# senweaver/senweaver-ide

Measured on AMD Instinct MI355X. Metric: APO iterations/sec (beam=4, llama-3-8b scorer, bf16), higher is better.
Workload: dtype bf16; 1 GPU; model=llama-3-8b, global_batch=64, seq_len=2048, parallelism=dp1, beam_width=4, branch_factor=4, gradient_batch_size=4

## Files before the change

### senweaver_amd/models/llama.py

```python

from __future__ import annotations

import math
import os
from typing import TYPE_CHECKING, Callable, List, Optional

import torch

from .. import ops
from .config import ModelConfig

if TYPE_CHECKING:
    from ..engine.kvcache import PagedKVCache


class LlamaModel:
    def __init__(self, config: ModelConfig, device="cpu", dtype=torch.bfloat16, seed: int = 0,
                 tp=None, quant: str = "bf16", ep=None):
        from ..parallel.tp import TPContext, shard_gateup, shard_qkv, shard_rows
        from ..parallel.ep import EPContext
        self.config = config
        self.device = torch.device(device)
        self.dtype = dtype
        self.tp = tp if tp is not None else TPContext()
# ... 168 lines not shown
    def plan_tensors(self, plan):
        cache = self._plan_cache
        key = (plan.S, plan.owner, plan.skip)
        hit = cache.get(key)
        if hit is None:
            if len(cache) >= 64:
                cache.clear()
            pos = torch.cat([torch.arange(plan.skip[b], plan.S)
                             for b in range(plan.B)])
            row = torch.repeat_interleave(
                torch.arange(plan.B),
                torch.tensor([plan.S - s for s in plan.skip]))
            hit = tuple(t.to(self.device) for t in (
                torch.tensor(plan.skip, dtype=torch.int32),
                torch.tensor(plan.base, dtype=torch.int32),
                torch.tensor(plan.owner, dtype=torch.int32),
                pos.to(torch.int32), row * plan.S + pos))
            cache[key] = hit
        return hit

    def prefill_packed(self, tokens: torch.Tensor, plan) -> torch.Tensor:
        c = self.config
        B, S = tokens.shape
        skip, base, owner, positions, flat_idx = self.plan_tensors(plan)
        Tp = plan.Tp
        if plan.is_identity or (self.device.type == "cuda"
                                and (S % 128 != 0 or S < 256)):
            return self.prefill(tokens).reshape(B * S, -1)[flat_idx]

        def attend(li, L, qkv):
            qb, kb = ops.rope_scatter_qkv_packed(
                qkv, self.cos_sin, positions, self.local_heads,
                self.local_kv_heads, c.head_dim, B, S, skip, base, owner)
            vt = ops.vt_from_qkv_packed(qkv, self.local_heads,
                                        self.local_kv_heads, c.head_dim, B, S,
                                        skip, base, owner)
            attn = ops.attn_fwd_packed(qb, kb, vt, self.scale, skip, base, Tp,
                                       flat_idx)
            if self.quant == "bf16" and not attn.is_cuda:
                return torch.matmul(attn, L["o"].t())
            return self._linear(attn, L, "o")

        hidden = self.embed[tokens.reshape(B * S)[flat_idx]]
        return self._layers(hidden, attend, full_rows=B * S)

    def _down_rows(self, h: torch.Tensor, L: dict, full_rows: int) -> Optional[int]:
        Tp = h.shape[0]
        if self.quant != "bf16" or "down" not in L or full_rows <= Tp:
            return None
        cache = self._down_rows_cache
        hit = cache.get((Tp, full_rows), 0)
        if hit == 0:
            hit = full_rows
            if h.is_cuda:
                w = L["down"]
                act = torch.empty(full_rows, w.shape[1], dtype=h.dtype,
                                  device=h.device).normal_()
                act[Tp:].zero_()
                t_packed = ops.gemm_lt_best_us(act[:Tp], w)
                t_full = ops.gemm_lt_best_us(act, w)
                if t_packed is not None and t_full is not None:
                    fill = ops.hip_ext().gemm_lt_fill_us(
                        act, (full_rows - Tp) * w.shape[1] * act.element_size())
                    if t_packed <= 1.05 * (t_full + fill):
                        hit = None
                elif torch.cuda.is_current_stream_capturing():
                    return full_rows
            if len(cache) >= 64:
                cache.clear()
            cache[(Tp, full_rows)] = hit
        return hit
# ... 251 lines not shown
```

### senweaver_amd/ops/__init__.py

```python

from __future__ import annotations

import math
import os
import weakref
from typing import Optional

import torch

from . import reference as ref

_ext = None
_ext_err: Optional[str] = None


def _load_ext():
    global _ext, _ext_err
    if _ext is not None or _ext_err is not None:
        return _ext
    from . import build as _build

    try:
        _ext = _build.load_prebuilt()
        if _ext is None:
# ... 112 lines not shown
    src = ref.packed_src_rows_ref(B, S, skip, base, owner).reshape(-1)
    return rope_scatter_qkv(qkv[src], cos_sin, positions[src], Hq, Hk, D, B, S)


def vt_from_qkv_packed(qkv: torch.Tensor, Hq: int, Hk: int, D: int, B: int,
                       S: int, skip, base, owner) -> torch.Tensor:
    if _on_gpu(qkv):
        return hip_ext().vt_from_qkv_packed(qkv.contiguous(), Hq, Hk, D, B, S,
                                            skip, base, owner)
    src = ref.packed_src_rows_ref(B, S, skip, base, owner).reshape(-1)
    return vt_from_qkv(qkv[src], Hq, Hk, D, B, S)


def attn_fwd_t_packed(q: torch.Tensor, k: torch.Tensor, vt: torch.Tensor,
                      scale: float, skip, base, Tp: int, flat_idx) -> torch.Tensor:
    B, H, S, D = q.shape
    if _on_gpu(q) and _ATTN_IMPL != "v2" and ((S + 255) // 256) * B * H >= 512:
        return hip_ext().attn_fwd_v5_packed(q.contiguous(), k.contiguous(),
                                            vt.contiguous(), scale, skip, base,
                                            Tp)
    ot = attn_fwd_t(q, k, vt, scale)
    return ot.permute(1, 2, 0, 3).reshape(H * D, B * S).index_select(1, flat_idx)


def attn_fwd_packed(q: torch.Tensor, k: torch.Tensor, vt: torch.Tensor,
                    scale: float, skip, base, Tp: int, flat_idx) -> torch.Tensor:
    B, H, S, D = q.shape
    if _on_gpu(q) and _ATTN_IMPL != "v2" and ((S + 255) // 256) * B * H >= 512:
        return hip_ext().attn_fwd_v5_packed_rm(q.contiguous(), k.contiguous(),
                                               vt.contiguous(), scale, skip,
                                               base, Tp)
    ot = attn_fwd_t(q, k, vt, scale)
    return ot.permute(0, 3, 1, 2).reshape(B * S, H * D).index_select(0, flat_idx)


def swiglu(gateup: torch.Tensor, out_rows: Optional[int] = None) -> torch.Tensor:
    if out_rows is not None and out_rows > gateup.shape[0]:
        if _on_gpu(gateup):
            return hip_ext().swiglu_padded(gateup.contiguous(), out_rows)
        act = ref.swiglu_ref(gateup)
        return torch.nn.functional.pad(act, (0, 0, 0, out_rows - act.shape[0]))
    if _on_gpu(gateup):
        return hip_ext().swiglu(gateup.contiguous())
    return ref.swiglu_ref(gateup)


_GEMM_IMPL = os.environ.get("SENWEAVER_GEMM", "auto")
_GEMM_TUNE = os.environ.get("SENWEAVER_GEMM_TUNE", "1") != "0"
_ATTN_IMPL = os.environ.get("SENWEAVER_ATTN", "auto")


def swiglu_gemv(gateup: torch.Tensor, w_down: torch.Tensor) -> torch.Tensor:
    K = gateup.shape[-1] // 2
    if (_on_gpu(gateup) and gateup.shape[0] == 1 and K % 1024 == 0
            and 4096 < K <= 14336 and w_down.shape[0] % 8 == 0):
        return hip_ext().swiglu_gemv_bt(gateup.contiguous(), w_down.contiguous())
    act = swiglu(gateup)
    return gemm_bt(act, w_down)


def gemv_fp8w(x: torch.Tensor, w_q: torch.Tensor, w_s: torch.Tensor) -> torch.Tensor:
    K = x.shape[-1]
    if _on_gpu(x) and x.shape[0] <= 8 and K % 1024 == 0 and w_q.shape[0] % 4 == 0:
        return hip_ext().gemv_bt_fp8w(x.contiguous(), w_q.contiguous(),
                                      w_s.contiguous())
    wf = w_q.view(torch.float8_e4m3fn).float() * w_s.unsqueeze(1)
# ... 325 lines not shown
```

### senweaver_amd/ops/csrc/attention_v5.hip

```cpp

#include "common.h"
#include "kernels.h"

typedef __attribute__((ext_vector_type(8))) short short8;
typedef __attribute__((ext_vector_type(16))) float f32x16;

#define V5_KVBLK 64
#define V5_QBLK 256
#define V5_NT 512
#define V5_CHUNKS (V5_KVBLK * 16)
#define V5_KC (V5_CHUNKS / V5_NT)

static __device__ __forceinline__ const ushort* v5_src(
    const ushort* __restrict__ src, long long ld, int chunks_per_row, int row,
    int cl) {
  const int c = (cl ^ row) & (chunks_per_row - 1);
  return src + (long long)row * ld + c * 8;
}

static __device__ __forceinline__ void v5_glds(const ushort* g,
                                               ushort* lds_wave) {
  __builtin_amdgcn_global_load_lds(
      (const __attribute__((address_space(1))) unsigned int*)g,
      (__attribute__((address_space(3))) unsigned int*)lds_wave, 16, 0, 0);
}

static __device__ __forceinline__ short8 v5_read(const ushort* lds_tile,
                                                 int row, int c,
                                                 int chunks_per_row) {
  const int phys = (c ^ row) & (chunks_per_row - 1);
  return *reinterpret_cast<const short8*>(lds_tile + (row * chunks_per_row + phys) * 8);
}

static __device__ __forceinline__ unsigned v5_cvt_pk_bf16(float lo, float hi) {
  unsigned r;
  asm("v_cvt_pk_bf16_f32 %0, %1, %2" : "=v"(r) : "v"(lo), "v"(hi));
  return r;
}

static __device__ __forceinline__ float v5_max(float a, float b) {
  float r;
  asm("v_max_f32 %0, %1, %2" : "=v"(r) : "v"(a), "v"(b));
  return r;
}

static __device__ __forceinline__ float v5_exp2(float x) {
  float r;
  asm("v_exp_f32 %0, %1" : "=v"(r) : "v"(x));
  return r;
}

template <int PACK>
static __device__ __forceinline__ void attn5_body(
    const ushort* __restrict__ Q, const ushort* __restrict__ K,
    const ushort* __restrict__ VT, ushort* __restrict__ OT, int B, int H,
    int Hk, int S, float scale, const int* __restrict__ pk_skip = nullptr,
    const int* __restrict__ pk_base = nullptr, int Tp = 0) {
  const int qb = gridDim.x - 1 - blockIdx.x;
  const int h = blockIdx.y;
  const int b = blockIdx.z;
  int skip = 0;
  if (PACK) {
    skip = pk_skip[b];
    if (qb * V5_QBLK + V5_QBLK <= skip) return;
  }
  const int kvh = h / (H / Hk);
  const int D = 128;

  const ushort* Qh = Q + (((long long)b * H + h) * S) * D;
  const ushort* Kh = K + (((long long)b * Hk + kvh) * S) * D;
  const ushort* VTh = VT + (((long long)b * Hk + kvh) * D) * S;
  ushort* OTh = OT + (((long long)b * H + h) * D) * S;

  const int tid = threadIdx.x;
  const int wid = tid >> 6;
  const int lane = tid & 63;
  const int l31 = lane & 31;
  const int lhi = lane >> 5;
  const int q0 = qb * V5_QBLK + wid * 32;
  const int q_lane = q0 + l31;
  const bool live = q_lane < S;

  __shared__ __attribute__((aligned(16))) ushort smem[2][V5_KVBLK * 128 + 128 * V5_KVBLK];

  short8 qf[8];
  {
    const long long qrow = (long long)(live ? q_lane : 0) * D;
#pragma unroll
    for (int st = 0; st < 8; ++st)
      qf[st] = *reinterpret_cast<const short8*>(Qh + qrow + st * 16 + lhi * 8);
  }

  float m_run = -INFINITY, l_run = 0.f;
  f32x16 o_acc[4];
#pragma unroll
  for (int db = 0; db < 4; ++db)
#pragma unroll
    for (int r = 0; r < 16; ++r) o_acc[db][r] = 0.f;

  const int kv_end = min(S, qb * V5_QBLK + V5_QBLK);
  for (int s0 = 0; s0 < V5_CHUNKS; s0 += V5_NT) {
    const int s = s0 + tid;
    if (s >= V5_CHUNKS) break;
    v5_glds(v5_src(Kh, D, 16, s / 16, s % 16),
            smem[0] + (long long)(s0 + (tid & ~63)) * 8);
  }
  for (int s0 = 0; s0 < V5_CHUNKS; s0 += V5_NT) {
    const int s = s0 + tid;
    if (s >= V5_CHUNKS) break;
    v5_glds(v5_src(VTh, S, 8, s / 8, s % 8),
            smem[0] + V5_KVBLK * 128 + (long long)(s0 + (tid & ~63)) * 8);
  }
  __syncthreads();
  int buf = 0;
  for (int kv0 = 0; kv0 < kv_end; kv0 += V5_KVBLK) {
    const bool more = kv0 + V5_KVBLK < kv_end;
    const ushort* k_lds = smem[buf];
    const ushort* vt_lds = smem[buf] + V5_KVBLK * 128;

    __builtin_amdgcn_s_setprio(1);
    f32x16 st[2];
#pragma unroll
    for (int sub = 0; sub < 2; ++sub) {
      f32x16 acc;
#pragma unroll
      for (int r = 0; r < 16; ++r) acc[r] = 0.f;
#pragma unroll
      for (int stp = 0; stp < 8; ++stp) {
        short8 kf = v5_read(k_lds, sub * 32 + l31, stp * 2 + lhi, 16);
        acc = __builtin_amdgcn_mfma_f32_32x32x16_bf16(kf, qf[stp], acc, 0, 0, 0);
      }
      st[sub] = acc;
    }
    __builtin_amdgcn_s_setprio(0);

    short8 stg[2 * V5_KC];
    if (more) {
      const ushort* Kn = Kh + (long long)(kv0 + V5_KVBLK) * D;
      const ushort* VTn = VTh + kv0 + V5_KVBLK;
#pragma unroll
      for (int c = 0; c < V5_KC; ++c) {
        const int s = tid + c * V5_NT;
        stg[c] = *reinterpret_cast<const short8*>(v5_src(Kn, D, 16, s / 16, s % 16));
        stg[V5_KC + c] = *reinterpret_cast<const short8*>(v5_src(VTn, S, 8, s / 8, s % 8));
      }
    }

    float vals[32];
    float tile_max = -INFINITY;
    const float scl = scale * 1.44269504f;
    const bool interior = kv0 + V5_KVBLK - 1 <= q0;
    if (interior) {
#pragma unroll
      for (int sub = 0; sub < 2; ++sub)
#pragma unroll
        for (int r = 0; r < 16; ++r) {
          const float v = st[sub][r] * scl;
          vals[sub * 16 + r] = v;
          tile_max = v5_max(tile_max, v);
        }
    } else {
#pragma unroll
      for (int sub = 0; sub < 2; ++sub)
#pragma unroll
        for (int r = 0; r < 16; ++r) {
          const int kv = kv0 + sub * 32 + (r & 3) + 8 * (r >> 2) + 4 * lhi;
          float v = st[sub][r] * scl;
          if (kv > q_lane) v = -INFINITY;
          vals[sub * 16 + r] = v;
          tile_max = v5_max(tile_max, v);
        }
    }
    tile_max = v5_max(tile_max, __shfl_xor(tile_max, 32, 64));
    const bool defer = __all((int)(tile_max - m_run <= 11.54f));
    float m_new, alpha;
    if (defer) {
      m_new = m_run;
      alpha = 1.f;
    } else {
      m_new = fmaxf(m_run, tile_max);
      alpha = (m_run == -INFINITY) ? 0.f : v5_exp2(m_run - m_new);
    }
    float rsum = 0.f;
    m_run = m_new;
    if (!defer) {
#pragma unroll
      for (int db = 0; db < 4; ++db)
#pragma unroll
        for (int r = 0; r < 16; ++r) o_acc[db][r] *= alpha;
    }

    if (more) {
      ushort* kd = smem[buf ^ 1];
      ushort* vd = smem[buf ^ 1] + V5_KVBLK * 128;
#pragma unroll
      for (int c = 0; c < V5_KC; ++c) {
        *reinterpret_cast<short8*>(kd + (long long)(tid + c * V5_NT) * 8) = stg[c];
        *reinterpret_cast<short8*>(vd + (long long)(tid + c * V5_NT) * 8) = stg[V5_KC + c];
      }
    }

#pragma unroll
    for (int sub = 0; sub < 2; ++sub) {
#pragma unroll
      for (int g = 0; g < 2; ++g) {
        const int base = sub * 16 + g * 8;
        float p[8];
#pragma unroll
        for (int i = 0; i < 8; ++i) {
          p[i] = v5_exp2(vals[base + i] - m_new);
          rsum += p[i];
        }
        unsigned x0 = v5_cvt_pk_bf16(p[0], p[1]);
        unsigned y0 = v5_cvt_pk_bf16(p[4], p[5]);
        unsigned x1 = v5_cvt_pk_bf16(p[2], p[3]);
        unsigned y1 = v5_cvt_pk_bf16(p[6], p[7]);
        auto r0 = __builtin_amdgcn_permlane32_swap(x0, y0, false, false);
        auto r1 = __builtin_amdgcn_permlane32_swap(x1, y1, false, false);
        short8 pfrag;
        unsigned* pw = reinterpret_cast<unsigned*>(&pfrag);
        pw[0] = (unsigned)r0[0];
        pw[1] = (unsigned)r1[0];
        pw[2] = (unsigned)r0[1];
        pw[3] = (unsigned)r1[1];
        const int kvg = sub * 32 + g * 16;
        __builtin_amdgcn_s_setprio(1);
#pragma unroll
        for (int db = 0; db < 4; ++db) {
          short8 vf = v5_read(vt_lds, db * 32 + l31, (kvg >> 3) + lhi, 8);
          o_acc[db] = __builtin_amdgcn_mfma_f32_32x32x16_bf16(vf, pfrag, o_acc[db], 0, 0, 0);
        }
        __builtin_amdgcn_s_setprio(0);
      }
    }
    rsum += __shfl_xor(rsum, 32, 64);
    l_run = l_run * alpha + rsum;

    __syncthreads();
    buf ^= 1;
  }

  const float inv_l = (l_run > 0.f) ? 1.f / l_run : 0.f;
  if (!live) return;
  if (PACK) {
    const long long col = (long long)pk_base[b] + q_lane;
    if (q_lane < skip || col < 0 || col >= Tp) return;
    if (PACK == 2) {
      ushort* Op = OT + col * ((long long)H * D) + h * D + 4 * lhi;
#pragma unroll
      for (int db = 0; db < 4; ++db)
#pragma unroll
        for (int g = 0; g < 4; ++g) {
          ushort4 v;
          v.x = f2bf(o_acc[db][g * 4 + 0] * inv_l);
          v.y = f2bf(o_acc[db][g * 4 + 1] * inv_l);
          v.z = f2bf(o_acc[db][g * 4 + 2] * inv_l);
          v.w = f2bf(o_acc[db][g * 4 + 3] * inv_l);
          *reinterpret_cast<ushort4*>(Op + db * 32 + 8 * g) = v;
        }
      return;
    }
    ushort* OTp = OT + (long long)h * D * Tp + col;
#pragma unroll
    for (int db = 0; db < 4; ++db)
#pragma unroll
      for (int r = 0; r < 16; ++r) {
        const int d = db * 32 + (r & 3) + 8 * (r >> 2) + 4 * lhi;
        OTp[(long long)d * Tp] = f2bf(o_acc[db][r] * inv_l);
      }
// ... 4 lines not shown
#pragma unroll
    for (int r = 0; r < 16; ++r) {
      const int d = db * 32 + (r & 3) + 8 * (r >> 2) + 4 * lhi;
      OTh[(long long)d * S + q_lane] = f2bf(o_acc[db][r] * inv_l);
    }
}

extern "C" __global__ void __launch_bounds__(512)
attn_fwd_v5_kernel(const ushort* __restrict__ Q, const ushort* __restrict__ K,
                   const ushort* __restrict__ VT, ushort* __restrict__ OT,
                   int B, int H, int Hk, int S, float scale) {
  attn5_body<0>(Q, K, VT, OT, B, H, Hk, S, scale);
}

extern "C" __global__ void __launch_bounds__(512)
attn_fwd_v5_packed_kernel(const ushort* __restrict__ Q,
                          const ushort* __restrict__ K,
                          const ushort* __restrict__ VT,
                          ushort* __restrict__ OT, int B, int H, int Hk,
                          int S, float scale, const int* __restrict__ skip,
                          const int* __restrict__ base, int Tp) {
  attn5_body<1>(Q, K, VT, OT, B, H, Hk, S, scale, skip, base, Tp);
}

extern "C" __global__ void __launch_bounds__(512)
attn_fwd_v5_packed_rm_kernel(const ushort* __restrict__ Q,
                             const ushort* __restrict__ K,
                             const ushort* __restrict__ VT,
                             ushort* __restrict__ O, int B, int H, int Hk,
                             int S, float scale, const int* __restrict__ skip,
                             const int* __restrict__ base, int Tp) {
  attn5_body<2>(Q, K, VT, O, B, H, Hk, S, scale, skip, base, Tp);
}
```

### senweaver_amd/ops/csrc/bindings.hip

```cpp

#include <torch/extension.h>
#include <c10/hip/HIPStream.h>
#include <hip/hip_runtime.h>

#include "common.h"
#include "kernels.h"

namespace {

inline hipStream_t cur_stream() {
  return c10::hip::getCurrentHIPStream().stream();
}

inline const ushort* bf16_ptr(const torch::Tensor& t) {
  return reinterpret_cast<const ushort*>(t.data_ptr());
}
inline ushort* bf16_mut(torch::Tensor& t) {
  return reinterpret_cast<ushort*>(t.data_ptr());
}

void check_bf16(const torch::Tensor& t, const char* name) {
  TORCH_CHECK(t.is_cuda(), name, " must be on GPU");
  TORCH_CHECK(t.scalar_type() == torch::kBFloat16, name, " must be bf16");
  TORCH_CHECK(t.is_contiguous(), name, " must be contiguous");
// ... 587 lines not shown
    ot = *out;
    check_bf16(ot, "out");
    TORCH_CHECK(ot.sizes().vec() == shape, "attn_fwd_v5_packed: out has the wrong shape");
    TORCH_CHECK((uintptr_t)ot.data_ptr() % 16 == 0, "attn_fwd_v5_packed: out must be 16-byte aligned");
  } else {
    ot = torch::empty(shape, q.options());
  }
  const dim3 grid((S + 255) / 256, H, B);
  if (row_major) {
    attn_fwd_v5_packed_rm_kernel<<<grid, dim3(512), 0, cur_stream()>>>(
        bf16_ptr(q), bf16_ptr(k), bf16_ptr(vt), bf16_mut(ot), B, H, Hk, S,
        (float)scale, skip.data_ptr<int>(), base.data_ptr<int>(), (int)Tp);
  } else {
    attn_fwd_v5_packed_kernel<<<grid, dim3(512), 0, cur_stream()>>>(
        bf16_ptr(q), bf16_ptr(k), bf16_ptr(vt), bf16_mut(ot), B, H, Hk, S,
        (float)scale, skip.data_ptr<int>(), base.data_ptr<int>(), (int)Tp);
  }
  HIP_CHECK_KERNEL();
  return ot;
}

torch::Tensor attn_fwd_v5_packed(torch::Tensor q, torch::Tensor k,
                                 torch::Tensor vt, double scale,
                                 torch::Tensor skip, torch::Tensor base,
                                 int64_t Tp) {
  return attn_packed_launch(q, k, vt, scale, skip, base, Tp, false, c10::nullopt);
}

torch::Tensor attn_fwd_v5_packed_rm(torch::Tensor q, torch::Tensor k,
                                    torch::Tensor vt, double scale,
                                    torch::Tensor skip, torch::Tensor base,
                                    int64_t Tp, c10::optional<torch::Tensor> out) {
  return attn_packed_launch(q, k, vt, scale, skip, base, Tp, true, out);
}

torch::Tensor paged_decode_attn(torch::Tensor q, torch::Tensor kcache,
                                torch::Tensor vcache, torch::Tensor block_table,
                                torch::Tensor ctx_lens, double scale) {
  check_bf16(q, "q");
  check_bf16(kcache, "kcache");
  check_bf16(vcache, "vcache");
  TORCH_CHECK(block_table.scalar_type() == torch::kInt32 && block_table.is_contiguous());
  TORCH_CHECK(ctx_lens.scalar_type() == torch::kInt32 && ctx_lens.is_contiguous());
  const int B = q.size(0), H = q.size(1), D = q.size(2);
  const int Hk = kcache.size(2);
  TORCH_CHECK(D == 128 && kcache.size(3) == D);
  TORCH_CHECK(kcache.size(1) == 16, "PAGE_SIZE=16");
  const int max_pages = block_table.size(1);
  auto o = torch::empty_like(q);
  auto partials = torch::empty({B, H, 8, 2 + 128},
                               q.options().dtype(torch::kFloat32));
  paged_decode_attn_partial_kernel<<<dim3(H, B, 8), dim3(256), 0, cur_stream()>>>(
      bf16_ptr(q), bf16_ptr(kcache), bf16_ptr(vcache),
      partials.data_ptr<float>(),
      block_table.data_ptr<int>(), ctx_lens.data_ptr<int>(), H, Hk, max_pages,
      (float)scale);
  paged_decode_attn_merge_kernel<<<dim3(H, B), dim3(64), 0, cur_stream()>>>(
      partials.data_ptr<float>(), bf16_mut(o), H);
  HIP_CHECK_KERNEL();
  return o;
}

torch::Tensor paged_prefill_attn(torch::Tensor q, torch::Tensor kcache,
                                 torch::Tensor vcache, torch::Tensor block_table,
                                 torch::Tensor ctx_lens, torch::Tensor q_lens,
                                 double scale) {
// ... 162 lines not shown
    return C;
  }, "fused silu(g)*u + streaming GEMV (decode down-proj, M=1)");
  m.def("grouped_gemm_bt", &grouped_gemm_bt, "segment-grouped C = A @ W[e]^T (MoE)");
  m.def("moe_combine", [](torch::Tensor down, torch::Tensor pos, torch::Tensor weight) {
    check_bf16(down, "down");
    TORCH_CHECK(pos.scalar_type() == torch::kInt32 && pos.dim() == 2);
    TORCH_CHECK(weight.scalar_type() == torch::kFloat32);
    const long long T = pos.size(0);
    const int k = pos.size(1), H = down.size(1);
    TORCH_CHECK(H % 8 == 0);
    auto out = torch::empty({T, (long)H}, down.options());
    moe_combine_kernel<<<dim3((unsigned)T), dim3(256), 0, cur_stream()>>>(
        bf16_ptr(down), pos.data_ptr<int>(), weight.data_ptr<float>(),
        bf16_mut(out), H, k);
    HIP_CHECK_KERNEL();
    return out;
  }, "routed-FFN weighted combine via inverse permutation");
  m.def("quant_fp8", &quant_fp8, "row-wise bf16 -> e4m3 + scale");
  m.def("gemm_bt_fp8", &gemm_bt_fp8, "fp8 MFMA GEMM with row/col rescale");
  m.def("quant_mxfp8", &quant_mxfp8, "OCP MX quant: bf16 -> e4m3 + e8m0 per-32 scales");
  m.def("gemm_bt_mxfp8", &gemm_bt_mxfp8, "MX block-scaled fp8 MFMA GEMM (32x32x64)");
  m.def("attn_fwd", &attn_fwd, "causal flash attention fwd (D=128, GQA)");
  m.def("attn_fwd_v2", &attn_fwd_v2, "swapped-QK^T attention; O^T out [B,H,D,S]");
  m.def("attn_fwd_v3", &attn_fwd_v3, "v2 with 8-wave shared K/V tiles; O^T out");
  m.def("attn_fwd_v5", &attn_fwd_v5, "production attention; O^T out");
  m.def("rope_scatter_qkv_packed", &rope_scatter_qkv_packed,
        "rope_scatter_qkv reading prefix-packed qkv rows");
  m.def("vt_from_qkv_packed", &vt_from_qkv_packed,
        "vt_from_qkv reading prefix-packed qkv rows");
  m.def("attn_fwd_v5_packed_rm", &attn_fwd_v5_packed_rm,
        "packed attention, row-major O [Tp, H*D]", pybind11::arg("q"), pybind11::arg("k"),
        pybind11::arg("vt"), pybind11::arg("scale"), pybind11::arg("skip"),
        pybind11::arg("base"), pybind11::arg("Tp"), pybind11::arg("out") = pybind11::none());
  m.def("attn_fwd_v5_packed", &attn_fwd_v5_packed,
        "attn_fwd_v5 skipping shared-prefix query rows; packed O^T [H*D, Tp] out");
  m.def("paged_decode_attn", &paged_decode_attn, "paged decode attention");
  m.def("paged_prefill_attn", &paged_prefill_attn,
        "prefill attention over the paged cache, queries at an offset");
  m.def("argmax_rows", &argmax_rows, "row argmax over bf16 logits");
  m.def("target_logprob", &target_logprob, "fused log_softmax gather");
}
```

### senweaver_amd/ops/csrc/common.h

```cpp
#pragma once

#include <hip/hip_runtime.h>
#include <hip/hip_bf16.h>
#include <hip/hip_fp16.h>

#define WAVE_SIZE 64

using bf16_t = __hip_bfloat16;

struct alignas(16) bf16x8 {
  ushort v[8];
};

struct alignas(8) bf16x4 {
  ushort v[4];
};

__device__ __forceinline__ float bf2f(ushort u) {
  union {
    unsigned int i;
    float f;
  } c;
  c.i = (unsigned int)u << 16;
  return c.f;
// ... 6 lines not shown
  } c;
  c.f = f;
  unsigned int lsb = (c.i >> 16) & 1u;
  unsigned int rounded = c.i + 0x7fffu + lsb;
  return (ushort)(rounded >> 16);
}

__device__ __forceinline__ float wave_reduce_sum(float v) {
#pragma unroll
  for (int off = 32; off > 0; off >>= 1) v += __shfl_xor(v, off, 64);
  return v;
}

__device__ __forceinline__ float wave_reduce_max(float v) {
#pragma unroll
  for (int off = 32; off > 0; off >>= 1) v = fmaxf(v, __shfl_xor(v, off, 64));
  return v;
}

template <int N>
__device__ __forceinline__ float group_reduce_sum(float v) {
#pragma unroll
  for (int off = N / 2; off > 0; off >>= 1) v += __shfl_xor(v, off, 64);
  return v;
}

template <int N>
__device__ __forceinline__ float group_reduce_max(float v) {
#pragma unroll
  for (int off = N / 2; off > 0; off >>= 1) v = fmaxf(v, __shfl_xor(v, off, 64));
  return v;
}

#define HIP_CHECK_KERNEL()                                     \
  do {                                                         \
    hipError_t e = hipGetLastError();                          \
    if (e != hipSuccess) {                                     \
      TORCH_CHECK(false, "HIP kernel launch failed: ",         \
                  hipGetErrorString(e));                       \
    }                                                          \
  } while (0)
```

### senweaver_amd/ops/csrc/elemwise.hip

```cpp

#include "common.h"
#include "kernels.h"

extern "C" __global__ void __launch_bounds__(256)
rmsnorm_fwd_kernel(const ushort* __restrict__ x, const ushort* __restrict__ w,
                   ushort* __restrict__ y, ushort* __restrict__ residual,
                   int hidden, float eps) {
  const int row = blockIdx.x;
  const long long base = (long long)row * hidden;
  const int nvec = hidden / 8;
  const bool fuse_res = residual != nullptr;

  float ss = 0.f;
  for (int i = threadIdx.x; i < nvec; i += blockDim.x) {
    bf16x8 v = *reinterpret_cast<const bf16x8*>(x + base + i * 8);
    if (fuse_res) {
      bf16x8 r = *reinterpret_cast<const bf16x8*>(residual + base + i * 8);
#pragma unroll
      for (int j = 0; j < 8; ++j) v.v[j] = f2bf(bf2f(v.v[j]) + bf2f(r.v[j]));
      *reinterpret_cast<bf16x8*>(residual + base + i * 8) = v;
    }
#pragma unroll
    for (int j = 0; j < 8; ++j) {
      float f = bf2f(v.v[j]);
// ... 17 lines not shown
    bf16x8 wv = *reinterpret_cast<const bf16x8*>(w + i * 8);
    bf16x8 out;
#pragma unroll
    for (int j = 0; j < 8; ++j)
      out.v[j] = f2bf(bf2f(v.v[j]) * inv_rms * bf2f(wv.v[j]));
    *reinterpret_cast<bf16x8*>(y + base + i * 8) = out;
  }
}

extern "C" __global__ void __launch_bounds__(64)
rope_fwd_kernel(ushort* __restrict__ q, ushort* __restrict__ k,
                const float* __restrict__ cos_sin,
                const int* __restrict__ positions, int Hq, int Hk, int D) {
  const int t = blockIdx.x;
  const int h = blockIdx.y;
  const int half = D / 2;
  ushort* ptr;
  if (h < Hq) {
    ptr = q + ((long long)t * Hq + h) * D;
  } else {
    ptr = k + ((long long)t * Hk + (h - Hq)) * D;
  }
  const float* cs = cos_sin + (long long)positions[t] * D;
  for (int d = threadIdx.x; d < half; d += blockDim.x) {
    float c = cs[d];
    float s = cs[half + d];
    float x1 = bf2f(ptr[d]);
    float x2 = bf2f(ptr[d + half]);
    ptr[d] = f2bf(x1 * c - x2 * s);
    ptr[d + half] = f2bf(x2 * c + x1 * s);
  }
}

static __device__ __forceinline__ long long packed_src_row(
    int b, int s, int B, const int* __restrict__ skip,
    const int* __restrict__ base, const int* __restrict__ owner) {
  int src_b = b;
  if (s < skip[b]) src_b = owner[b];
  if ((unsigned)src_b >= (unsigned)B) return -1;
  return (long long)base[src_b] + s;
}

template <bool PACKED>
static __device__ __forceinline__ void rope_scatter_body(
    const ushort* __restrict__ qkv, long long ld,
    ushort* __restrict__ q_out, ushort* __restrict__ k_out,
    const float* __restrict__ cos_sin,
    const int* __restrict__ positions, int Hq, int Hk, int D,
    int S, int B, const int* __restrict__ skip, const int* __restrict__ base,
    const int* __restrict__ owner, long long Tp) {
  const int t = blockIdx.x;
  const int half = D / 2;
  const int lanes_per_head = half / 8;
  const int heads_per_blk = 256 / lanes_per_head;
  const int h = blockIdx.y * heads_per_blk + threadIdx.x / lanes_per_head;
  if (h >= Hq + Hk) return;
  const int b = t / S;
  const int s = t % S;
  long long tr = t;
  if (PACKED) {
    tr = packed_src_row(b, s, B, skip, base, owner);
    if (tr < 0 || tr >= Tp) return;
  }
  const ushort* src;
  ushort* dst;
  if (h < Hq) {
    src = qkv + tr * ld + (long long)h * D;
    dst = q_out + (((long long)b * Hq + h) * S + s) * D;
  } else {
    src = qkv + tr * ld + (long long)Hq * D + (long long)(h - Hq) * D;
    dst = k_out + (((long long)b * Hk + (h - Hq)) * S + s) * D;
  }
  const float* cs = cos_sin + (long long)positions[tr] * D;
  const int d0 = (threadIdx.x % lanes_per_head) * 8;
// ... 203 lines not shown
```

### senweaver_amd/ops/csrc/kernels.h

```cpp
#pragma once

#include "common.h"

#define SW_KERNEL extern "C" __global__ void

SW_KERNEL rmsnorm_fwd_kernel(const ushort* x, const ushort* w, ushort* y,
                             ushort* residual, int hidden, float eps);
SW_KERNEL rope_fwd_kernel(ushort* q, ushort* k, const float* cos_sin,
                          const int* positions, int Hq, int Hk, int D);
SW_KERNEL rope_scatter_kernel(const ushort* qkv, long long ld, ushort* q_out,
                              ushort* k_out, const float* cos_sin,
                              const int* positions, int Hq, int Hk, int D, int S);
SW_KERNEL rope_scatter_packed_kernel(const ushort* qkv, long long ld,
                                     ushort* q_out, ushort* k_out,
                                     const float* cos_sin, const int* positions,
                                     int Hq, int Hk, int D, int S, int B,
                                     const int* skip, const int* base,
                                     const int* owner, long long Tp);
SW_KERNEL transpose_v_kernel(const ushort* qkv, long long ld, long long v_off,
                             ushort* vt, int B, int S, int Hk, int D);
SW_KERNEL transpose_v_packed_kernel(const ushort* qkv, long long ld,
                                    long long v_off, ushort* vt, int B, int S,
                                    int Hk, int D, const int* skip,
                                    const int* base, const int* owner,
// ... 88 lines not shown
                             ushort* C, int M, int N, int K);
SW_KERNEL quant_mxfp8_kernel(const ushort* x, unsigned char* q,
                             unsigned char* scales, int K);
SW_KERNEL gemm_bt_mxfp8_kernel(const unsigned char* A, const unsigned char* As,
                               const unsigned char* B, const unsigned char* Bs,
                               ushort* C, int M, int N, int K);
SW_KERNEL gemm_bt_mxfp8_256_kernel(const unsigned char* A,
                                   const unsigned char* As,
                                   const unsigned char* B,
                                   const unsigned char* Bs, ushort* C, int M,
                                   int N, int K);

SW_KERNEL attn_fwd_bf16_kernel(const ushort* Q, const ushort* K,
                               const ushort* VT, ushort* O, int B, int H,
                               int Hk, int S, float scale);
SW_KERNEL attn_fwd_v2_kernel(const ushort* Q, const ushort* K, const ushort* VT,
                             ushort* OT, int B, int H, int Hk, int S,
                             float scale);
SW_KERNEL attn_fwd_v3_kernel(const ushort* Q, const ushort* K, const ushort* VT,
                             ushort* OT, int B, int H, int Hk, int S,
                             float scale);
SW_KERNEL attn_fwd_v5_kernel(const ushort* Q, const ushort* K, const ushort* VT,
                             ushort* OT, int B, int H, int Hk, int S,
                             float scale);
SW_KERNEL attn_fwd_v5_packed_kernel(const ushort* Q, const ushort* K,
                                    const ushort* VT, ushort* OT, int B, int H,
                                    int Hk, int S, float scale, const int* skip,
                                    const int* base, int Tp);
SW_KERNEL attn_fwd_v5_packed_rm_kernel(const ushort* Q, const ushort* K,
                                       const ushort* VT, ushort* O, int B,
                                       int H, int Hk, int S, float scale,
                                       const int* skip, const int* base,
                                       int Tp);

SW_KERNEL paged_decode_attn_partial_kernel(const ushort* Q, const ushort* Kcache,
                                           const ushort* Vcache, float* partials,
                                           const int* block_table,
                                           const int* ctx_lens, int H, int Hk,
                                           int max_pages, float scale);
SW_KERNEL paged_decode_attn_merge_kernel(const float* partials, ushort* O,
                                         int H);
SW_KERNEL paged_prefill_attn_kernel(const ushort* Q, const ushort* Kcache,
                                    const ushort* Vcache, ushort* O,
                                    const int* block_table, const int* ctx_lens,
                                    const int* q_lens, int Sq, int H, int Hk,
                                    int max_pages, float scale);

#undef SW_KERNEL
```

Before: 0.7171 iterations/s.

## Read V directly from packed qkv rows in attention, dropping V transpose

```diff
diff --git a/senweaver_amd/models/llama.py b/senweaver_amd/models/llama.py
--- a/senweaver_amd/models/llama.py
+++ b/senweaver_amd/models/llama.py
@@ -224,11 +224,9 @@
             qb, kb = ops.rope_scatter_qkv_packed(
                 qkv, self.cos_sin, positions, self.local_heads,
                 self.local_kv_heads, c.head_dim, B, S, skip, base, owner)
-            vt = ops.vt_from_qkv_packed(qkv, self.local_heads,
-                                        self.local_kv_heads, c.head_dim, B, S,
-                                        skip, base, owner)
-            attn = ops.attn_fwd_packed(qb, kb, vt, self.scale, skip, base, Tp,
-                                       flat_idx)
+            attn = ops.attn_fwd_packed_qkv(
+                qb, kb, qkv, self.local_heads, self.local_kv_heads,
+                c.head_dim, self.scale, skip, base, owner, Tp, flat_idx)
             if self.quant == "bf16" and not attn.is_cuda:
                 return torch.matmul(attn, L["o"].t())
             return self._linear(attn, L, "o")
diff --git a/senweaver_amd/ops/__init__.py b/senweaver_amd/ops/__init__.py
--- a/senweaver_amd/ops/__init__.py
+++ b/senweaver_amd/ops/__init__.py
@@ -168,6 +168,18 @@
                                                base, Tp)
     ot = attn_fwd_t(q, k, vt, scale)
     return ot.permute(0, 3, 1, 2).reshape(B * S, H * D).index_select(0, flat_idx)
+
+
+def attn_fwd_packed_qkv(qb: torch.Tensor, kb: torch.Tensor, qkv: torch.Tensor,
+                        Hq: int, Hk: int, D: int, scale: float, skip, base,
+                        owner, Tp: int, flat_idx) -> torch.Tensor:
+    B, H, S, _ = qb.shape
+    if _on_gpu(qb) and _ATTN_IMPL != "v2" and ((S + 255) // 256) * B * H >= 512:
+        return hip_ext().attn_fwd_v5_packed_rm_qkv(
+            qb.contiguous(), kb.contiguous(), qkv.contiguous(), Hq, Hk, scale,
+            skip, base, owner, Tp)
+    vt = vt_from_qkv_packed(qkv, Hq, Hk, D, B, S, skip, base, owner)
+    return attn_fwd_packed(qb, kb, vt, scale, skip, base, Tp, flat_idx)
 
 
 def swiglu(gateup: torch.Tensor, out_rows: Optional[int] = None) -> torch.Tensor:
diff --git a/senweaver_amd/ops/csrc/attention_v5.hip b/senweaver_amd/ops/csrc/attention_v5.hip
--- a/senweaver_amd/ops/csrc/attention_v5.hip
+++ b/senweaver_amd/ops/csrc/attention_v5.hip
@@ -3,6 +3,7 @@
 #include "kernels.h"
 
 typedef __attribute__((ext_vector_type(8))) short short8;
+typedef __attribute__((ext_vector_type(4))) short short4v;
 typedef __attribute__((ext_vector_type(16))) float f32x16;
 
 #define V5_KVBLK 64
@@ -32,6 +33,26 @@
   return *reinterpret_cast<const short8*>(lds_tile + (row * chunks_per_row + phys) * 8);
 }
 
+static __device__ __forceinline__ int v5_vx(int r) {
+  return ((r & 3) << 2) | ((r >> 2) & 3);
+}
+
+static __device__ __forceinline__ short8 v5_read_tr(const ushort* v_lds,
+                                                    int lane, int kvg, int db) {
+  const int p = lane & 3, q = (lane >> 2) & 3, hh = (lane >> 4) & 1;
+  const int lhi = lane >> 5;
+  short4v part[2];
+#pragma unroll
+  for (int j = 0; j < 2; ++j) {
+    const int row = kvg + 8 * lhi + 4 * j + q;
+    const int ch = db * 4 + 2 * hh + (p >> 1);
+    const int off = row * 128 + (ch ^ v5_vx(row)) * 8 + 4 * (p & 1);
+    part[j] = __builtin_amdgcn_ds_read_tr16_b64_v4i16(
+        (__attribute__((address_space(3))) short4v*)(v_lds + off));
+  }
+  return __builtin_shufflevector(part[0], part[1], 0, 1, 2, 3, 4, 5, 6, 7);
+}
+
 static __device__ __forceinline__ unsigned v5_cvt_pk_bf16(float lo, float hi) {
   unsigned r;
   asm("v_cvt_pk_bf16_f32 %0, %1, %2" : "=v"(r) : "v"(lo), "v"(hi));
@@ -50,15 +71,41 @@
   return r;
 }
 
-template <int PACK>
+static __device__ __forceinline__ void attn5_xcd_block(int B, int H, int Hk,
+                                                       int nqb, int& qb,
+                                                       int& h, int& b) {
+  const int i = blockIdx.x;
+  const int groups = B * Hk;
+  if (groups % 8 == 0) {
+    const int rep = H / Hk;
+    const int per_rank = (groups / 8) * rep;
+    const int j = i / 8;
+    const int r = j % per_rank;
+    const int g = i % 8 + 8 * (r / rep);
+    qb = nqb - 1 - j / per_rank;
+    h = (g % Hk) * rep + r % rep;
+    b = g / Hk;
+  } else {
+    qb = nqb - 1 - i % nqb;
+    h = (i / nqb) % H;
+    b = i / (nqb * H);
+  }
+}
+
+template <int PACK, bool VROWS = false>
 static __device__ __forceinline__ void attn5_body(
     const ushort* __restrict__ Q, const ushort* __restrict__ K,
     const ushort* __restrict__ VT, ushort* __restrict__ OT, int B, int H,
     int Hk, int S, float scale, const int* __restrict__ pk_skip = nullptr,
-    const int* __restrict__ pk_base = nullptr, int Tp = 0) {
-  const int qb = gridDim.x - 1 - blockIdx.x;
-  const int h = blockIdx.y;
-  const int b = blockIdx.z;
+    const int* __restrict__ pk_base = nullptr, int Tp = 0,
+    const int* __restrict__ pk_owner = nullptr, long long ld = 0,
+    long long v_off = 0, long long Tq = 0) {
+  static_assert(!VROWS || PACK == 2, "VROWS reads packed qkv rows");
+  constexpr bool WSKIP = VROWS, XCD = VROWS;
+  int qb = gridDim.x - 1 - blockIdx.x;
+  int h = blockIdx.y;
+  int b = blockIdx.z;
+  if (XCD) attn5_xcd_block(B, H, Hk, (S + V5_QBLK - 1) / V5_QBLK, qb, h, b);
   int skip = 0;
   if (PACK) {
     skip = pk_skip[b];
@@ -69,7 +116,20 @@
 
   const ushort* Qh = Q + (((long long)b * H + h) * S) * D;
   const ushort* Kh = K + (((long long)b * Hk + kvh) * S) * D;
-  const ushort* VTh = VT + (((long long)b * Hk + kvh) * D) * S;
+  const ushort* VTh = VROWS ? VT + v_off + (long long)kvh * D
+                             : VT + (((long long)b * Hk + kvh) * D) * S;
+  long long pre0 = 0, own0 = 0;
+  if (VROWS) {
+    pre0 = packed_src_row(b, 0, B, pk_skip, pk_base, pk_owner);
+    own0 = pk_base[b];
+  }
+  auto v_rows_src = [&](int kv0, int s) -> const ushort* {
+    const int r = s >> 4;
+    const int key = kv0 + r;
+    long long tr = (key < skip ? pre0 : own0) + key;
+    if ((key < skip && pre0 < 0) || tr < 0 || tr >= Tq) tr = 0;
+    return VTh + tr * ld + ((s & 15) ^ v5_vx(r)) * 8;
+  };
   ushort* OTh = OT + (((long long)b * H + h) * D) * S;
 
   const int tid = threadIdx.x;
@@ -79,6 +139,7 @@
   const int lhi = lane >> 5;
   const int q0 = qb * V5_QBLK + wid * 32;
   const int q_lane = q0 + l31;
+  const int q0_wave = qb * V5_QBLK + __builtin_amdgcn_readfirstlane(wid) * 32;
   const bool live = q_lane < S;
 
   __shared__ __attribute__((aligned(16))) ushort smem[2][V5_KVBLK * 128 + 128 * V5_KVBLK];
@@ -108,7 +169,7 @@
   for (int s0 = 0; s0 < V5_CHUNKS; s0 += V5_NT) {
     const int s = s0 + tid;
     if (s >= V5_CHUNKS) break;
-    v5_glds(v5_src(VTh, S, 8, s / 8, s % 8),
+    v5_glds(VROWS ? v_rows_src(0, s) : v5_src(VTh, S, 8, s / 8, s % 8),
             smem[0] + V5_KVBLK * 128 + (long long)(s0 + (tid & ~63)) * 8);
   }
   __syncthreads();
@@ -117,22 +178,25 @@
     const bool more = kv0 + V5_KVBLK < kv_end;
     const ushort* k_lds = smem[buf];
     const ushort* vt_lds = smem[buf] + V5_KVBLK * 128;
-
-    __builtin_amdgcn_s_setprio(1);
+    const bool work = !WSKIP || kv0 <= q0_wave + 31;
+
     f32x16 st[2];
-#pragma unroll
-    for (int sub = 0; sub < 2; ++sub) {
-      f32x16 acc;
-#pragma unroll
-      for (int r = 0; r < 16; ++r) acc[r] = 0.f;
-#pragma unroll
-      for (int stp = 0; stp < 8; ++stp) {
-        short8 kf = v5_read(k_lds, sub * 32 + l31, stp * 2 + lhi, 16);
-        acc = __builtin_amdgcn_mfma_f32_32x32x16_bf16(kf, qf[stp], acc, 0, 0, 0);
-      }
-      st[sub] = acc;
-    }
-    __builtin_amdgcn_s_setprio(0);
+    if (work) {
+      __builtin_amdgcn_s_setprio(1);
+#pragma unroll
+      for (int sub = 0; sub < 2; ++sub) {
+        f32x16 acc;
+#pragma unroll
+        for (int r = 0; r < 16; ++r) acc[r] = 0.f;
+#pragma unroll
+        for (int stp = 0; stp < 8; ++stp) {
+          short8 kf = v5_read(k_lds, sub * 32 + l31, stp * 2 + lhi, 16);
+          acc = __builtin_amdgcn_mfma_f32_32x32x16_bf16(kf, qf[stp], acc, 0, 0, 0);
+        }
+        st[sub] = acc;
+      }
+      __builtin_amdgcn_s_setprio(0);
+    }
 
     short8 stg[2 * V5_KC];
     if (more) {
@@ -142,52 +206,51 @@
       for (int c = 0; c < V5_KC; ++c) {
         const int s = tid + c * V5_NT;
         stg[c] = *reinterpret_cast<const short8*>(v5_src(Kn, D, 16, s / 16, s % 16));
-        stg[V5_KC + c] = *reinterpret_cast<const short8*>(v5_src(VTn, S, 8, s / 8, s % 8));
+        stg[V5_KC + c] = *reinterpret_cast<const short8*>(
+            VROWS ? v_rows_src(kv0 + V5_KVBLK, s) : v5_src(VTn, S, 8, s / 8, s % 8));
       }
     }
 
     float vals[32];
-    float tile_max = -INFINITY;
-    const float scl = scale * 1.44269504f;
-    const bool interior = kv0 + V5_KVBLK - 1 <= q0;
-    if (interior) {
-#pragma unroll
-      for (int sub = 0; sub < 2; ++sub)
-#pragma unroll
-        for (int r = 0; r < 16; ++r) {
-          const float v = st[sub][r] * scl;
-          vals[sub * 16 + r] = v;
-          tile_max = v5_max(tile_max, v);
-        }
-    } else {
-#pragma unroll
-      for (int sub = 0; sub < 2; ++sub)
-#pragma unroll
-        for (int r = 0; r < 16; ++r) {
-          const int kv = kv0 + sub * 32 + (r & 3) + 8 * (r >> 2) + 4 * lhi;
-          float v = st[sub][r] * scl;
-          if (kv > q_lane) v = -INFINITY;
-          vals[sub * 16 + r] = v;
-          tile_max = v5_max(tile_max, v);
-        }
-    }
-    tile_max = v5_max(tile_max, __shfl_xor(tile_max, 32, 64));
-    const bool defer = __all((int)(tile_max - m_run <= 11.54f));
-    float m_new, alpha;
-    if (defer) {
-      m_new = m_run;
-      alpha = 1.f;
-    } else {
-      m_new = fmaxf(m_run, tile_max);
-      alpha = (m_run == -INFINITY) ? 0.f : v5_exp2(m_run - m_new);
-    }
-    float rsum = 0.f;
-    m_run = m_new;
-    if (!defer) {
-#pragma unroll
-      for (int db = 0; db < 4; ++db)
-#pragma unroll
-        for (int r = 0; r < 16; ++r) o_acc[db][r] *= alpha;
+    float m_new = m_run, alpha = 1.f;
+    if (work) {
+      float tile_max = -INFINITY;
+      const float scl = scale * 1.44269504f;
+      const bool interior = kv0 + V5_KVBLK - 1 <= q0;
+      if (interior) {
+#pragma unroll
+        for (int sub = 0; sub < 2; ++sub)
+#pragma unroll
+          for (int r = 0; r < 16; ++r) {
+            const float v = st[sub][r] * scl;
+            vals[sub * 16 + r] = v;
+            tile_max = v5_max(tile_max, v);
+          }
+      } else {
+#pragma unroll
+        for (int sub = 0; sub < 2; ++sub)
+#pragma unroll
+          for (int r = 0; r < 16; ++r) {
+            const int kv = kv0 + sub * 32 + (r & 3) + 8 * (r >> 2) + 4 * lhi;
+            float v = st[sub][r] * scl;
+            if (kv > q_lane) v = -INFINITY;
+            vals[sub * 16 + r] = v;
+            tile_max = v5_max(tile_max, v);
+          }
+      }
+      tile_max = v5_max(tile_max, __shfl_xor(tile_max, 32, 64));
+      const bool defer = __all((int)(tile_max - m_run <= 11.54f));
+      if (!defer) {
+        m_new = fmaxf(m_run, tile_max);
+        alpha = (m_run == -INFINITY) ? 0.f : v5_exp2(m_run - m_new);
+      }
+      m_run = m_new;
+      if (!defer) {
+#pragma unroll
+        for (int db = 0; db < 4; ++db)
+#pragma unroll
+          for (int r = 0; r < 16; ++r) o_acc[db][r] *= alpha;
+      }
     }
 
     if (more) {
@@ -200,41 +263,45 @@
       }
     }
 
-#pragma unroll
-    for (int sub = 0; sub < 2; ++sub) {
-#pragma unroll
-      for (int g = 0; g < 2; ++g) {
-        const int base = sub * 16 + g * 8;
-        float p[8];
-#pragma unroll
-        for (int i = 0; i < 8; ++i) {
-          p[i] = v5_exp2(vals[base + i] - m_new);
-          rsum += p[i];
+    if (work) {
+      float rsum = 0.f;
+#pragma unroll
+      for (int sub = 0; sub < 2; ++sub) {
+#pragma unroll
+        for (int g = 0; g < 2; ++g) {
+          const int base = sub * 16 + g * 8;
+          float p[8];
+#pragma unroll
+          for (int i = 0; i < 8; ++i) {
+            p[i] = v5_exp2(vals[base + i] - m_new);
+            rsum += p[i];
+          }
+          unsigned x0 = v5_cvt_pk_bf16(p[0], p[1]);
+          unsigned y0 = v5_cvt_pk_bf16(p[4], p[5]);
+          unsigned x1 = v5_cvt_pk_bf16(p[2], p[3]);
+          unsigned y1 = v5_cvt_pk_bf16(p[6], p[7]);
+          auto r0 = __builtin_amdgcn_permlane32_swap(x0, y0, false, false);
+          auto r1 = __builtin_amdgcn_permlane32_swap(x1, y1, false, false);
+          short8 pfrag;
+          unsigned* pw = reinterpret_cast<unsigned*>(&pfrag);
+          pw[0] = (unsigned)r0[0];
+          pw[1] = (unsigned)r1[0];
+          pw[2] = (unsigned)r0[1];
+          pw[3] = (unsigned)r1[1];
+          const int kvg = sub * 32 + g * 16;
+          __builtin_amdgcn_s_setprio(1);
+#pragma unroll
+          for (int db = 0; db < 4; ++db) {
+            short8 vf = VROWS ? v5_read_tr(vt_lds, lane, kvg, db)
+                              : v5_read(vt_lds, db * 32 + l31, (kvg >> 3) + lhi, 8);
+            o_acc[db] = __builtin_amdgcn_mfma_f32_32x32x16_bf16(vf, pfrag, o_acc[db], 0, 0, 0);
+          }
+          __builtin_amdgcn_s_setprio(0);
         }
-        unsigned x0 = v5_cvt_pk_bf16(p[0], p[1]);
-        unsigned y0 = v5_cvt_pk_bf16(p[4], p[5]);
-        unsigned x1 = v5_cvt_pk_bf16(p[2], p[3]);
-        unsigned y1 = v5_cvt_pk_bf16(p[6], p[7]);
-        auto r0 = __builtin_amdgcn_permlane32_swap(x0, y0, false, false);
-        auto r1 = __builtin_amdgcn_permlane32_swap(x1, y1, false, false);
-        short8 pfrag;
-        unsigned* pw = reinterpret_cast<unsigned*>(&pfrag);
-        pw[0] = (unsigned)r0[0];
-        pw[1] = (unsigned)r1[0];
-        pw[2] = (unsigned)r0[1];
-        pw[3] = (unsigned)r1[1];
-        const int kvg = sub * 32 + g * 16;
-        __builtin_amdgcn_s_setprio(1);
-#pragma unroll
-        for (int db = 0; db < 4; ++db) {
-          short8 vf = v5_read(vt_lds, db * 32 + l31, (kvg >> 3) + lhi, 8);
-          o_acc[db] = __builtin_amdgcn_mfma_f32_32x32x16_bf16(vf, pfrag, o_acc[db], 0, 0, 0);
-        }
-        __builtin_amdgcn_s_setprio(0);
-      }
-    }
-    rsum += __shfl_xor(rsum, 32, 64);
-    l_run = l_run * alpha + rsum;
+      }
+      rsum += __shfl_xor(rsum, 32, 64);
+      l_run = l_run * alpha + rsum;
+    }
 
     __syncthreads();
     buf ^= 1;
@@ -305,3 +372,17 @@
                              const int* __restrict__ base, int Tp) {
   attn5_body<2>(Q, K, VT, O, B, H, Hk, S, scale, skip, base, Tp);
 }
+
+extern "C" __global__ void __launch_bounds__(512)
+attn_fwd_v5_packed_rm_qkv_kernel(const ushort* __restrict__ Q,
+                                 const ushort* __restrict__ K,
+                                 const ushort* __restrict__ qkv, long long ld,
+                                 long long v_off, long long Tq,
+                                 ushort* __restrict__ O, int B, int H, int Hk,
+                                 int S, float scale,
+                                 const int* __restrict__ skip,
+                                 const int* __restrict__ base,
+                                 const int* __restrict__ owner, int Tp) {
+  attn5_body<2, true>(Q, K, qkv, O, B, H, Hk, S, scale, skip, base, Tp, owner,
+                      ld, v_off, Tq);
+}
diff --git a/senweaver_amd/ops/csrc/bindings.hip b/senweaver_amd/ops/csrc/bindings.hip
--- a/senweaver_amd/ops/csrc/bindings.hip
+++ b/senweaver_amd/ops/csrc/bindings.hip
@@ -643,6 +643,52 @@
                                     torch::Tensor skip, torch::Tensor base,
                                     int64_t Tp, c10::optional<torch::Tensor> out) {
   return attn_packed_launch(q, k, vt, scale, skip, base, Tp, true, out);
+}
+
+torch::Tensor attn_fwd_v5_packed_rm_qkv(torch::Tensor q, torch::Tensor k,
+                                        torch::Tensor qkv, int64_t Hq,
+                                        int64_t Hk, double scale,
+                                        torch::Tensor skip, torch::Tensor base,
+                                        torch::Tensor owner, int64_t Tp,
+                                        c10::optional<torch::Tensor> out) {
+  check_bf16(q, "q");
+  check_bf16(k, "k");
+  check_bf16(qkv, "qkv");
+  TORCH_CHECK(q.dim() == 4 && k.dim() == 4 && qkv.dim() == 2,
+              "attn_fwd_v5_packed_rm_qkv: q [B,H,S,D], k [B,Hk,S,D], qkv [Tq,ld]");
+  const int64_t B = q.size(0), S = q.size(2), D = q.size(3);
+  TORCH_CHECK(q.size(1) == Hq && Hk > 0 && Hq % Hk == 0 && D == 128 && S % 128 == 0,
+              "attn_fwd_v5_packed_rm_qkv: needs D == 128, S % 128 == 0, Hq % Hk == 0");
+  TORCH_CHECK(k.size(0) == B && k.size(1) == Hk && k.size(2) == S && k.size(3) == D,
+              "attn_fwd_v5_packed_rm_qkv: k must be [B,Hk,S,D]");
+  const long long Tq = qkv.size(0);
+  const long long ld = qkv.size(1);
+  TORCH_CHECK(Tq > 0 && Tq <= B * S && ld % 8 == 0 && ld >= (Hq + 2 * Hk) * D,
+              "attn_fwd_v5_packed_rm_qkv: qkv must hold (0, B*S] rows of at least "
+              "(Hq+2Hk)*D columns, row length a multiple of 8");
+  TORCH_CHECK(Tp > 0 && Tp <= B * S && B * S < (1LL << 31),
+              "attn_fwd_v5_packed_rm_qkv: Tp must be in (0, B*S]");
+  check_plan(skip, B, "skip");
+  check_plan(base, B, "base");
+  check_plan(owner, B, "owner");
+  const std::vector<int64_t> shape{Tp, Hq * D};
+  torch::Tensor o;
+  if (out.has_value()) {
+    o = *out;
+    check_bf16(o, "out");
+    TORCH_CHECK(o.sizes().vec() == shape, "attn_fwd_v5_packed_rm_qkv: out has the wrong shape");
+    TORCH_CHECK((uintptr_t)o.data_ptr() % 16 == 0, "attn_fwd_v5_packed_rm_qkv: out must be 16-byte aligned");
+  } else {
+    o = torch::empty(shape, q.options());
+  }
+  const long long v_off = (Hq + Hk) * D;
+  const int nqb = (int)((S + 255) / 256);
+  attn_fwd_v5_packed_rm_qkv_kernel<<<dim3((unsigned)(nqb * Hq * B)), dim3(512), 0, cur_stream()>>>(
+      bf16_ptr(q), bf16_ptr(k), bf16_ptr(qkv), ld, v_off, Tq, bf16_mut(o),
+      (int)B, (int)Hq, (int)Hk, (int)S, (float)scale, skip.data_ptr<int>(),
+      base.data_ptr<int>(), owner.data_ptr<int>(), (int)Tp);
+  HIP_CHECK_KERNEL();
+  return o;
 }
 
 torch::Tensor paged_decode_attn(torch::Tensor q, torch::Tensor kcache,
@@ -871,6 +917,12 @@
         "packed attention, row-major O [Tp, H*D]", pybind11::arg("q"), pybind11::arg("k"),
         pybind11::arg("vt"), pybind11::arg("scale"), pybind11::arg("skip"),
         pybind11::arg("base"), pybind11::arg("Tp"), pybind11::arg("out") = pybind11::none());
+  m.def("attn_fwd_v5_packed_rm_qkv", &attn_fwd_v5_packed_rm_qkv,
+        "packed attention reading V from the packed qkv rows, row-major O [Tp, Hq*D]",
+        pybind11::arg("q"), pybind11::arg("k"), pybind11::arg("qkv"), pybind11::arg("Hq"),
+        pybind11::arg("Hk"), pybind11::arg("scale"), pybind11::arg("skip"),
+        pybind11::arg("base"), pybind11::arg("owner"), pybind11::arg("Tp"),
+        pybind11::arg("out") = pybind11::none());
   m.def("attn_fwd_v5_packed", &attn_fwd_v5_packed,
         "attn_fwd_v5 skipping shared-prefix query rows; packed O^T [H*D, Tp] out");
   m.def("paged_decode_attn", &paged_decode_attn, "paged decode attention");
diff --git a/senweaver_amd/ops/csrc/common.h b/senweaver_amd/ops/csrc/common.h
--- a/senweaver_amd/ops/csrc/common.h
+++ b/senweaver_amd/ops/csrc/common.h
@@ -62,6 +62,15 @@
   return v;
 }
 
+static __device__ __forceinline__ long long packed_src_row(
+    int b, int s, int B, const int* __restrict__ skip,
+    const int* __restrict__ base, const int* __restrict__ owner) {
+  int src_b = b;
+  if (s < skip[b]) src_b = owner[b];
+  if ((unsigned)src_b >= (unsigned)B) return -1;
+  return (long long)base[src_b] + s;
+}
+
 #define HIP_CHECK_KERNEL()                                     \
   do {                                                         \
     hipError_t e = hipGetLastError();                          \
diff --git a/senweaver_amd/ops/csrc/elemwise.hip b/senweaver_amd/ops/csrc/elemwise.hip
--- a/senweaver_amd/ops/csrc/elemwise.hip
+++ b/senweaver_amd/ops/csrc/elemwise.hip
@@ -73,14 +73,6 @@
   }
 }
 
-static __device__ __forceinline__ long long packed_src_row(
-    int b, int s, int B, const int* __restrict__ skip,
-    const int* __restrict__ base, const int* __restrict__ owner) {
-  int src_b = b;
-  if (s < skip[b]) src_b = owner[b];
-  if ((unsigned)src_b >= (unsigned)B) return -1;
-  return (long long)base[src_b] + s;
-}
 
 template <bool PACKED>
 static __device__ __forceinline__ void rope_scatter_body(
diff --git a/senweaver_amd/ops/csrc/kernels.h b/senweaver_amd/ops/csrc/kernels.h
--- a/senweaver_amd/ops/csrc/kernels.h
+++ b/senweaver_amd/ops/csrc/kernels.h
@@ -144,6 +144,13 @@
                                        int H, int Hk, int S, float scale,
                                        const int* skip, const int* base,
                                        int Tp);
+SW_KERNEL attn_fwd_v5_packed_rm_qkv_kernel(const ushort* Q, const ushort* K,
+                                           const ushort* qkv, long long ld,
+                                           long long v_off, long long Tq,
+                                           ushort* O, int B, int H, int Hk,
+                                           int S, float scale, const int* skip,
+                                           const int* base, const int* owner,
+                                           int Tp);
 
 SW_KERNEL paged_decode_attn_partial_kernel(const ushort* Q, const ushort* Kcache,
                                            const ushort* Vcache, float* partials,
```

New measurement: 0.7477 iterations/s (median of 6 runs). 4.3% higher.
